# microsoft/gated-graph-neural-network-samples

Hardware: AMD Instinct MI355X
Metric: node-state updates/sec on QM9-shaped graphs, h=100, 4 edge types (higher is better)
Workload: dtype f32

## Files before the change

### gated-graph-neural-network-samples_amd/csrc/ggnn_common.h

```cpp
#pragma once
#include <hip/hip_runtime.h>
#include <atomic>
#include <cstdarg>
#include <cstdio>
#include "../../include/ggnn_hip.h"

namespace ggnn {

typedef float f32x4 __attribute__((ext_vector_type(4)));

constexpr int kNumXcd = 8;

char* error_buffer();
int fail(int code, const char* fmt, ...);

#define GGNN_CHECK_ARG(cond, ...) \
    do { if (!(cond)) return ::ggnn::fail(GGNN_E_INVALID, __VA_ARGS__); } while (0)

#define GGNN_CHECK_HIP(expr)                                                                   \
    do {                                                                                       \
        hipError_t e_ = (expr);                                                                \
        if (e_ != hipSuccess)                                                                  \
            return ::ggnn::fail(GGNN_E_HIP, "%s failed: %s", #expr, hipGetErrorString(e_));    \
    } while (0)

inline bool aligned16(const void* p) { return (reinterpret_cast<uintptr_t>(p) & 15u) == 0; }

int num_cus();

int stream_order_after(hipStream_t waiter, hipStream_t producer);

template <class Kernel>
inline hipError_t allow_dynamic_lds(Kernel* kernel, size_t bytes, std::atomic<unsigned long long>& done) {
    int dev = 0;
    if (hipError_t e = hipGetDevice(&dev); e != hipSuccess) return e;
    const unsigned long long bit = 1ULL << (dev & 63);
    if (done.load(std::memory_order_acquire) & bit) return hipSuccess;
    if (hipError_t e = hipFuncSetAttribute(reinterpret_cast<const void*>(kernel), hipFuncAttributeMaxDynamicSharedMemorySize,
                                           (int)bytes); e != hipSuccess) return e;
    done.fetch_or(bit, std::memory_order_release);
    return hipSuccess;
}

}
```

### gated-graph-neural-network-samples_amd/csrc/ggnn_gemm.hip

```cpp
#include "ggnn_gemm.hpp"

namespace ggnn {

static inline int round_up8(int x) { return (x + 7) / 8 * 8; }

constexpr int kPersistBlocksPerCU = 2;

template <int KC, int MT, int NT, int NW, class Epi>
static int launch_gemm(const GemmOperands& g, const Epi& epi, hipStream_t st) {
    using Cfg = GemmCfg<KC, MT, NT, NW>;
    const int ncg = (g.N + Cfg::BN - 1) / Cfg::BN;
    const int row_tiles = (g.M + Cfg::BM - 1) / Cfg::BM;
    if (row_tiles == 0 || ncg == 0) return GGNN_OK;
    const int nstages = g.nseg * (g.D / KC);
    int workers = round_up8(row_tiles);
    if (nstages == 1) {
        int target = num_cus() * kPersistBlocksPerCU / ncg;
        target = target / 8 * 8;
        if (target < 8) target = 8;
        if (workers > target) workers = target;
    }
    const dim3 grid((unsigned)(ncg * workers));
    hipLaunchKernelGGL((ggnn_gemm_kernel<KC, MT, NT, NW, Epi>), grid, dim3(Cfg::THREADS), Cfg::LDS_BYTES, st,
                       g, epi, ncg, row_tiles, workers);
// ... 257 lines not shown
    GGNN_CHECK_ARG(aligned16(dY) && aligned16(WT), "pointers must be 16-byte aligned");
    GemmOperands g{};
    for (int s = 0; s < nseg_y; ++s) { g.A[s] = dY + (size_t)s * D; g.lda[s] = ldy; }
    g.nseg = nseg_y; g.D = D; g.M = V;
    g.B = WT; g.ldb = K; g.b_blk_cols = K; g.b_blk_stride = 0; g.N = K;
    const int inc0 = inc ? xcols - D : xcols;
    EpiBwdDx e{dx, xcols > 0 ? xcols : 4, xcols, inc0, dinc, nin, T, use_avg, dh, D, acc_dx, acc_dh};
    return dispatch_gemm(g, e, (hipStream_t)stream);
}

extern "C" int ggnn_gru_packed_gather_f32(const float* const* x_segs, int nx, const float* h, const float* packed,
                                          const float* bg, const float* bc, float* h_out, const float* Hrows,
                                          const int32_t* row_ptr, const int32_t* gather_row, const float* nin, int T, int use_avg,
                                          int V, int D, int act, int gru_fmt, int32_t* tile_counter, ggnn_stream_t stream) {
    return ggnn_gru_packed_gather_train_f32(x_segs, nx, h, packed, bg, bc, h_out, Hrows, row_ptr, gather_row, nin, T, use_avg,
                                            nullptr, nullptr, nullptr, nullptr, V, D, act, gru_fmt, tile_counter, stream);
}

extern "C" int ggnn_gru_packed_gather_train_f32(const float* const* x_segs, int nx, const float* h, const float* packed,
                                                const float* bg, const float* bc, float* h_out, const float* Hrows,
                                                const int32_t* row_ptr, const int32_t* gather_row, const float* nin, int T,
                                                int use_avg, float* save_r, float* save_u, float* save_c, float* save_incoming,
                                                int V, int D, int act, int gru_fmt, int32_t* tile_counter, ggnn_stream_t stream) {
    if (int rc = check_common(V, D)) return rc;
    if (int rc = gru_fmt_check(gru_fmt)) return rc;
    const bool save = save_r || save_u || save_c || save_incoming;
    GGNN_CHECK_ARG(!save || (save_r && save_u && save_c && save_incoming && aligned16(save_r) && aligned16(save_u) && aligned16(save_c) &&
                             aligned16(save_incoming)), "save_r / save_u / save_c / save_incoming must be given together, 16-byte aligned");
    GGNN_CHECK_ARG(nx >= 1 && nx <= 3, "nx %d outside 1..3", nx);
    GGNN_CHECK_ARG(act == GGNN_ACT_TANH || act == GGNN_ACT_RELU, "unknown activation %d", act);
    if (!gru_fused_supported(D)) return fail(GGNN_E_UNSUPPORTED, "no fused GRU for hidden size %d", D);
    if (V == 0) return GGNN_OK;
    GGNN_CHECK_ARG(h && packed && bg && bc && h_out && h_out != h && Hrows && row_ptr && T > 0, "null pointer or h_out aliases h");
    GGNN_CHECK_ARG(!use_avg || nin, "nin is required for mean aggregation");
    GGNN_CHECK_ARG(nx == 1 || x_segs, "residual segments missing");
    GGNN_CHECK_ARG(aligned16(h) && aligned16(packed) && aligned16(bg) && aligned16(bc) && aligned16(h_out) && aligned16(Hrows),
                   "pointers must be 16-byte aligned");
    GruFusedArgs a{};
    for (int s = 0; s + 1 < nx; ++s) {
        GGNN_CHECK_ARG(x_segs[s] && aligned16(x_segs[s]) && x_segs[s] != h_out, "residual segment %d null, misaligned or aliasing h_out", s);
        a.x[s] = x_segs[s];
    }
    a.nx = nx; a.h = h; a.bg = bg; a.bc = bc; a.h_out = h_out; a.V = V; a.act = act;
    a.save_r = save_r; a.save_u = save_u; a.save_c = save_c; a.save_x = save_incoming;
    a.g_H = Hrows; a.g_row_ptr = row_ptr; a.g_idx = gather_row; a.g_nin = nin; a.g_T = T; a.g_use_avg = use_avg;
    a.tickets = tile_counter; a.fmt = gru_fmt;
    return gru_fused_dispatch(a, D, const_cast<float*>(packed), (hipStream_t)stream);
}

extern "C" int ggnn_gru_bwd_dx_cand_f32(const float* dpc, const float* WcT, const float* h, const float* r, float* dx, float* dh,
                                        float* dpg, int nx, int V, int D, ggnn_stream_t stream) {
    if (int rc = check_common(V, D)) return rc;
    GGNN_CHECK_ARG(nx >= 1 && nx <= kGemmMaxSeg - 1, "nx %d outside 1..%d", nx, kGemmMaxSeg - 1);
    if (V == 0) return GGNN_OK;
    GGNN_CHECK_ARG(dpc && WcT && h && r && dx && dh && dpg, "null pointer");
    GGNN_CHECK_ARG(aligned16(dpc) && aligned16(WcT) && aligned16(h) && aligned16(r) && aligned16(dx) && aligned16(dh) && aligned16(dpg),
                   "pointers must be 16-byte aligned");
    const int K = (nx + 1) * D;
    GemmOperands g{};
    g.A[0] = dpc; g.lda[0] = D; g.nseg = 1; g.D = D; g.M = V;
    g.B = WcT; g.ldb = K; g.b_blk_cols = K; g.b_blk_stride = 0; g.N = K;
    EpiBwdCand e{dx, nx * D, nx * D, h, r, dh, dpg, D};
    return dispatch_gemm(g, e, (hipStream_t)stream);
}

extern "C" int ggnn_gru_bwd_dx_gates_f32(const float* dpg, const float* WgT, float* dx, float* dinc, const float* nin, int T,
                                         int use_avg, float* dh, int nx, int V, int D, ggnn_stream_t stream) {
    if (int rc = check_common(V, D)) return rc;
// ... 12 lines not shown
```

### gated-graph-neural-network-samples_amd/csrc/ggnn_gemm.hpp

```cpp
#pragma once
#include "ggnn_common.h"

namespace ggnn {

constexpr int kGemmMaxSeg = 8;
constexpr int kGruFusedMaxNx = 3;

struct GemmOperands {
    const float* A[kGemmMaxSeg];
    int lda[kGemmMaxSeg];
    int nseg;
    int D;
    const float* B;
    int ldb;
    int b_blk_cols;
    long b_blk_stride;
    int M, N;
};

__device__ __forceinline__ f32x4 ld4(const float* p) { return *reinterpret_cast<const f32x4*>(p); }
__device__ __forceinline__ void st4(float* p, f32x4 v) { *reinterpret_cast<f32x4*>(p) = v; }

__device__ __forceinline__ float sigmoid_f(float x) { return __builtin_amdgcn_rcpf(1.0f + __expf(-x)); }
__device__ __forceinline__ float tanh_f(float x) { return 1.0f - 2.0f * __builtin_amdgcn_rcpf(1.0f + __expf(2.0f * x)); }
// ... 125 lines not shown
            return;
        }
        f32x4 t = v;
        if (acc_dx) t = t + ld4(dx + (size_t)row * ld_dx + col);
        if (col < inc0) { st4(dx + (size_t)row * ld_dx + col, t); return; }
        if (use_avg) {
            float deg = 0.f;
            for (int k = 0; k < T; ++k) deg += nin[(size_t)row * T + k];
            t = t / (deg + 1e-7f);
        }
        st4(dinc + (size_t)row * D + (col - inc0), t);
    }
};

struct GruFusedArgs {
    const float* x[3];
    int nx;
    const float* h;
    const float* Wg; const float* bg; const float* Wc; const float* bc;
    float* h_out; float* save_r; float* save_u; float* save_c;
    float* save_x;
    int V; int act;
    const float* g_H; const int* g_row_ptr; const int* g_idx; const float* g_nin; int g_T; int g_use_avg;
    int* tickets;
    int fmt;
    unsigned long long* tdbg;
};

int gru_fused_supported(int D);
int gru_pack_floats(int D, int nx);
int gru_fused_dispatch(const GruFusedArgs& a, int D, float* packed, hipStream_t st);

template <int KC, int MT, int NT, int NW>
struct GemmCfg {
    static constexpr int BN = NT * 16;
    static constexpr int LDB = BN + 4;
    static constexpr int BM = NW * MT * 16;
    static constexpr int NC = KC / 16;
    static constexpr int NR = (KC % 16) / 4;
    static constexpr int THREADS = NW * 64;
    static constexpr int BVEC = (KC * (BN / 4) + THREADS - 1) / THREADS;
    static constexpr size_t LDS_BYTES = (size_t)KC * LDB * sizeof(float);
};

template <int KC, int MT, int NT, int NW, class Epi>
__global__ __launch_bounds__(NW * 64) void ggnn_gemm_kernel(GemmOperands g, Epi epi, int ncg,
// ... 135 lines not shown
```

### gated-graph-neural-network-samples_amd/csrc/ggnn_gru_fused.hip

```cpp
#include "ggnn_split.hpp"
#include <type_traits>

#ifndef GGNN_COOP_DEPTH
#define GGNN_COOP_DEPTH 1
#endif
#ifndef GGNN_GRU_STAMPS
#define GGNN_GRU_STAMPS 0
#endif
#if GGNN_GRU_STAMPS
#define GGNN_TDBG(a) (a).tdbg
#else
#define GGNN_TDBG(a) ((unsigned long long*)nullptr)
#endif

#ifndef GGNN_GRU_ABLATE
#define GGNN_GRU_ABLATE 0
#endif
#if GGNN_GRU_ABLATE
#define GGNN_ABL(BIT) ((ablate & (BIT)) != 0)
#define GGNN_ABL_PARAM , int ablate
#define GGNN_ABL_ARG , gru_ablate_bits()
static int gru_ablate_bits() { static const int v = [] { const char* e = getenv("GGNN_GRU_DBG"); return e ? atoi(e) : 0; }(); return v; }
#else
#define GGNN_ABL(BIT) (false)
#define GGNN_ABL_PARAM
#define GGNN_ABL_ARG
#endif

namespace ggnn {

constexpr int kTkRuntime = -1, kTkStatic = 0, kTkCounter = 1;

int gru_panel_supported(int D);
int gru_panel_pack_floats(int D, int nx);
int gru_panel_dispatch(const GruFusedArgs& a, int D, float* packed, hipStream_t st);

int gru_split_launch(int D, int nx, bool gather, const GruFusedArgs& a, float* packed, hipStream_t st);

#ifndef GGNN_GRU_TU_SPLIT
int gru_pack_floats(int D, int nx) {
    if (gru_panel_supported(D)) return gru_panel_pack_floats(D, nx);
    const bool sp = split_matrix_path();
    static_assert(ImgCfg<100, true>::IMG >= ImgCfg<100, true, kSplitF16x2>::IMG && ImgCfg<64, true>::IMG >= ImgCfg<64, true, kSplitF16x2>::IMG &&
                  ImgCfg<32, true>::IMG >= ImgCfg<32, true, kSplitF16x2>::IMG, "bf16x3 images are the larger ones");
    switch (D) {
        case 100: return 3 * (nx + 1) * (sp ? ImgCfg<100, true>::IMG : ImgCfg<100, false>::IMG);
        case 64: return 3 * (nx + 1) * (sp ? ImgCfg<64, true>::IMG : ImgCfg<64, false>::IMG);
        case 32: return 3 * (nx + 1) * (sp ? ImgCfg<32, true>::IMG : ImgCfg<32, false>::IMG);
        default: return 0;
    }
}
#endif

template <int D, bool SPLIT, int FMT = kSplitBf16x3>
// ... 10 lines not shown
    return (pos % 3) < 2 ? 2 * (pos / 3) + (pos % 3) : 2 * (NX + 1) + pos / 3;
}

template <int FMT>
__device__ __forceinline__ f32x4 sigmoid4_acc(f32x4 z, f32x4 b_scaled) {
    constexpr float k = -kLog2e * SplitFmt<FMT>::acc_scale;
    return rcp_4(exp2_4(z * k + b_scaled) + 1.0f);
}
template <int FMT>
__device__ __forceinline__ f32x4 tanh4_acc(f32x4 z, f32x4 b_scaled) {
    constexpr float k = 2.0f * kLog2e * SplitFmt<FMT>::acc_scale;
    return 1.0f - 2.0f * rcp_4(exp2_4(z * k + b_scaled) + 1.0f);
}

template <int D>
__device__ __forceinline__ void frag_zero(Frag<D>& f) {
#pragma unroll
    for (int c = 0; c < StageCfg<D>::NC; ++c) f.v[c] = f32x4{0.f, 0.f, 0.f, 0.f};
#pragma unroll
    for (int q = 0; q < StageCfg<D>::NR; ++q) f.r[q] = 0.f;
}

template <int D>
__device__ __forceinline__ void frag_add(Frag<D>& f, const Frag<D>& t) {
#pragma unroll
    for (int c = 0; c < StageCfg<D>::NC; ++c) f.v[c] += t.v[c];
#pragma unroll
    for (int q = 0; q < StageCfg<D>::NR; ++q) f.r[q] += t.r[q];
}

template <int D, int NX, int NW, bool SAVE, bool GATHER, bool SPLIT, bool SAVEX = SAVE, int FORM = 0, int FMT = kSplitBf16x3,
          int TK = kTkRuntime, bool G4AVG = false>
__global__ __launch_bounds__(NW * 64, FORM == 1 ? 2 : 1) void ggnn_gru_fused_kernel(GruFusedArgs a, const float* __restrict__ packed GGNN_ABL_PARAM) {
    static_assert(SPLIT || FMT == kSplitBf16x3, "the f32-MFMA kernels have no operand format");
    using C = StageCfg<D>;
    using I = ImgCfg<D, SPLIT, FMT>;
    using SC = SplitCfg<D, FMT>;
    constexpr bool HALF = FORM != 0;
    constexpr bool DEEP = FORM == 2;
    constexpr int NSLOT = DEEP ? 3 : 2;
    static_assert(!HALF || SPLIT, "the half-stage forms are split-form kernels");
    static_assert(FORM != 1 || NW == 4, "form 1 is the four-wave kernel");
    static_assert(!G4AVG || GATHER, "G4AVG fixes the gather's parameters");
    auto dyn_tk = [&]() -> bool {
        if constexpr (TK == kTkRuntime) return a.tickets != nullptr;
        else return TK == kTkCounter;
    };
    constexpr int NT = C::NT, NC = C::NC, NR = C::NR;
    constexpr int NSTAGE = 3 * (NX + 1);
    constexpr int SLOT = HALF ? SC::HA : I::IMG;
    extern __shared__ __attribute__((aligned(16))) float lds_[];

    const int tid = threadIdx.x, lane = tid & 63;
    const int wave = __builtin_amdgcn_readfirstlane(tid >> 6);
    const int li = lane & 15, kq = lane >> 4;
    if (GGNN_TDBG(a) && tid == 0) {
        a.tdbg[4096 + blockIdx.x * 4 + 0] = __builtin_amdgcn_s_memtime();
        a.tdbg[4096 + blockIdx.x * 4 + 1] = __builtin_amdgcn_s_memrealtime();
    }

    const int wt_total = (a.V + 15) / 16;
    const int nb = gridDim.x;
    const int full_tk = wt_total / (NW * nb) * nb;
    const int rest = wt_total - full_tk * NW;
    const int tail_w = (rest + nb - 1) / nb;
    const int n_tk = full_tk + (tail_w ? (rest + tail_w - 1) / tail_w : 0);
    const bool coop_tail = !HALF && (tail_w == 1) && (NT <= NW);
    auto is_coop = [&](int t) -> bool { return coop_tail && t >= full_tk && t < n_tk; };
    auto tile_of = [&](int t) -> int {
        if (t < full_tk) return t * NW + wave;
        if (t >= n_tk) return -1;
        if (coop_tail) return full_tk * NW + (t - full_tk);
        const int tl = full_tk * NW + (t - full_tk) * tail_w + wave;
        return (wave < tail_w && tl < wt_total) ? tl : -1;
    };

    constexpr int BIAS_FLOATS = (4 * D + 4 + 63) / 64 * 64;
    float* bias_s = lds_;
    float* ring = lds_ + BIAS_FLOATS;
    int* tk_slot = reinterpret_cast<int*>(bias_s + 4 * D);
    constexpr int RHP = C::BN + 4;
    float* rh_x = ring + NSLOT * SLOT;
    for (int i = tid; i < 4 * D; i += NW * 64)
        bias_s[i] = i < 2 * D ? -kLog2e * a.bg[i] : (i < 3 * D ? 2.0f * kLog2e * a.bc[i - 2 * D] : a.bc[i - 3 * D]);
    const bool late = FORM == 1 || wave >= NW / 2;
    int tk = blockIdx.x, tk_next = blockIdx.x + nb;
    if (dyn_tk() && tid == 0) *tk_slot = nb + atomicAdd(a.tickets, 1);

    int cur = 0;
    auto image_src = [&](int image) -> const float* {
        const float* p = packed;
        asm volatile("" : "+s"(p));
        return p + (size_t)image * I::IMG;
    };
    auto dma = [&](const float* src, float* dst) {
        if constexpr (SPLIT) dma_image_asm<I::IMG_BYTES, NW>(src, dst, wave, lane);
        else dma_image<I::IMG_BYTES, NW>(src, dst, wave, lane);
    };
    auto publish = [&]() { if constexpr (SPLIT) dma_wait(); __syncthreads(); };
    auto dma_ha = [&](const float* src, float* dst) { dma_kib_asm<SC::HA_BYTES / 1024, NW>(src, dst, wave, lane); };
    auto dma_hb = [&](const float* src, float* dst) { dma_kib_asm<SC::HB_BYTES / 1024, NW>(src, dst, wave, lane); };
    constexpr int KA = SC::HA_BYTES / 1024, KB = SC::HB_BYTES / 1024;
    const int own_a = KA / NW + (wave < KA % NW ? 1 : 0), own_b = KB / NW + (wave < KB % NW ? 1 : 0);
    auto publish_deep = [&](int own) {
        switch (own) {
            case 0: asm volatile("s_waitcnt vmcnt(0) lgkmcnt(0)" ::: "memory"); break;
// ... 2 lines not shown
            case 3: asm volatile("s_waitcnt vmcnt(3) lgkmcnt(0)" ::: "memory"); break;
            case 4: asm volatile("s_waitcnt vmcnt(4) lgkmcnt(0)" ::: "memory"); break;
            case 5: asm volatile("s_waitcnt vmcnt(5) lgkmcnt(0)" ::: "memory"); break;
            case 6: asm volatile("s_waitcnt vmcnt(6) lgkmcnt(0)" ::: "memory"); break;
            case 7: asm volatile("s_waitcnt vmcnt(7) lgkmcnt(0)" ::: "memory"); break;
            case 8: asm volatile("s_waitcnt vmcnt(8) lgkmcnt(0)" ::: "memory"); break;
            case 9: asm volatile("s_waitcnt vmcnt(9) lgkmcnt(0)" ::: "memory"); break;
            default: asm volatile("s_waitcnt vmcnt(10) lgkmcnt(0)" ::: "memory"); break;
        }
        __builtin_amdgcn_s_barrier();
    };
    static_assert(!DEEP || (SC::HA_BYTES / 1024 + NW - 1) / NW <= 10, "publish_deep covers <= 10 pieces per wave");
    if constexpr (DEEP) {
        dma_ha(packed, ring);
        dma_hb(packed + SC::HA, ring + SLOT);
    } else if constexpr (HALF) dma_ha(packed, ring);
    else dma(packed, ring);

    constexpr int GSEG = NX - 1, GBUF = GSEG & 1;
    constexpr int KI = 4;
    constexpr int G_U = NX == 1 ? NSTAGE : 3 * (NX - 1);
    constexpr bool G_NEXT = (NX == 1);
    int g_beg = 0, g_end = 0;
    int g_i[KI] = {0, 0, 0, 0};
    f32x4 g_n = {0.f, 0.f, 0.f, 0.f};
    float g_den = 1.f, g_rcp = 1.f;
    Frag<D> gt;

    auto g_ptrs = [&](int r, bool on) {
        const int b = ldi_b(a.g_row_ptr, (unsigned)r * 4u), e = ldi_b(a.g_row_ptr, (unsigned)r * 4u + 4u);
        g_beg = on ? b : 0; g_end = on ? e : 0;
        if constexpr (G4AVG) {
            g_n = ld4_b(a.g_nin, (unsigned)r * 16u);
        } else if (a.g_use_avg) {
            if (a.g_T == 4) {
                g_n = ld4_b(a.g_nin, (unsigned)r * 16u);
            } else {
                float deg = 0.f;
                for (int t = 0; t < a.g_T; ++t) deg += a.g_nin[(size_t)r * a.g_T + t];
                g_n = f32x4{deg, 0.f, 0.f, 0.f};
            }
        }
    };
    auto touch = [](auto v) { asm volatile("" :: "v"(v)); };
    auto g_index = [&](int part) {
        if (part != 2) {
            touch(g_beg); touch(g_end);
            g_den = (((g_n.x + g_n.y) + g_n.z) + g_n.w) + 1e-7f;
            if constexpr (NX == 1) g_rcp = 1.0f / g_den;
        }
        if (part != 1) {
#pragma unroll
            for (int j = 0; j < KI; ++j) {
                g_i[j] = 0;
                if (g_beg + j < g_end) g_i[j] = ldi_b(a.g_idx, (unsigned)(g_beg + j) * 4u);
            }
        }
    };
    auto g_rows0 = [&](Frag<D>& f, int part) {
        if (part != 2) { touch(g_i[0]); touch(g_i[1]); touch(g_i[2]); touch(g_i[3]); }
        if (part != 1) {
            load_frag<D>(f, a.g_H, g_i[0], kq);
            load_frag<D>(gt, a.g_H, g_i[1], kq);
        }
    };
    auto g_rows = [&](Frag<D>& f, int k, int part) {
        if (part != 2) { if (g_beg + k - 1 < g_end) frag_add<D>(f, gt); }
        if (part != 1) load_frag<D>(gt, a.g_H, g_i[k], kq);
    };
    auto g_finish = [&](Frag<D>& f) {
        if (g_beg + KI - 1 < g_end) frag_add<D>(f, gt);
        for (int e = g_beg + KI; e < g_end; ++e) {
            load_frag<D>(gt, a.g_H, a.g_idx[e], kq);
            frag_add<D>(f, gt);
        }
        if (g_beg >= g_end) frag_zero<D>(f);
        if (G4AVG || a.g_use_avg) {
            const float den = g_den, r = g_rcp;
            auto dv = [&](float x) {
                if constexpr (NX == 1) { const float q = x * r; return fmaf(fmaf(-den, q, x), r, q); }
                else return x / den;
            };
#pragma unroll
            for (int c = 0; c < NC; ++c) f.v[c] = f32x4{dv(f.v[c].x), dv(f.v[c].y), dv(f.v[c].z), dv(f.v[c].w)};
#pragma unroll
            for (int q = 0; q < NR; ++q) f.r[q] = dv(f.r[q]);
        }
    };

    auto store_x = [&](const Frag<D>& f, int row_) {
        const unsigned ob = ((unsigned)row_ * (unsigned)D + 4u * (unsigned)kq) * 4u;
#pragma unroll
        for (int c = 0; c < NC; ++c) st4_b(a.save_x, ob + 64u * c, f.v[c]);
#pragma unroll
        for (int q = 0; q < NR; ++q) *reinterpret_cast<float*>(reinterpret_cast<char*>(a.save_x) + ob - 16u * (unsigned)kq + (16u * NC + 4u * q + (unsigned)kq) * 4u) = f.r[q];
    };
    Frag<D> hf, xf[2];
    {
        const int t0 = tile_of(tk);
        const bool on = t0 >= 0;
        const int r0 = (on ? t0 : 0) * 16 + li;
        const int r0c = r0 < a.V ? r0 : a.V - 1;
        if constexpr (GATHER) {
// ... 285 lines not shown
#pragma unroll
            for (int c = 0; c < NC; ++c) rh.v[c] = acc_r[c] * hf.v[c];
#pragma unroll
            for (int q = 0; q < NR; ++q) {
                const float t0 = __shfl(acc_r[NT - 1].x, li + 16 * q), t1 = __shfl(acc_r[NT - 1].y, li + 16 * q);
                const float t2 = __shfl(acc_r[NT - 1].z, li + 16 * q), t3 = __shfl(acc_r[NT - 1].w, li + 16 * q);
                const float rr = kq == 0 ? t0 : (kq == 1 ? t1 : (kq == 2 ? t2 : t3));
                rh.r[q] = rr * hf.r[q];
            }
        }

        if (dyn_tk() && tid == 0) tk_slot[(p + 1) & 1] = nb + tk_fetch;
        GGNN_STAGE(3 * NX + 2, acc_c, rh)
#undef GGNN_STAGE
#undef GGNN_HALF_STAGE
#undef GGNN_COOP_STAGE
        tk = tk_next;
        tk_next = dyn_tk() ? __builtin_amdgcn_readfirstlane(tk_slot[(p + 1) & 1]) : tk_next + nb;

        if constexpr (coop) {
            const int col = wave * 16 + 4 * kq;
            if (wave < NT && col < D && row < a.V && !GGNN_ABL(4)) {
                f32x4 c;
                if (a.act == GGNN_ACT_TANH) {
                    c = tanh4_acc<FMT>(acc_c[0], ld4(bias_s + 2 * D + col));
                } else {
                    c = acc_c[0] * SplitFmt<FMT>::acc_scale + ld4(bias_s + 3 * D + col);
                    c.x = fmaxf(c.x, 0.f); c.y = fmaxf(c.y, 0.f); c.z = fmaxf(c.z, 0.f); c.w = fmaxf(c.w, 0.f);
                }
                const f32x4 u = acc_u[0], hv = acc_r[0];
                st4_b(a.h_out, ((unsigned)row * D + col) * 4u, u * hv + (1.0f - u) * c);
                if constexpr (SAVE) { if (a.save_c) st4_b(a.save_c, ((unsigned)row * D + col) * 4u, c); }
            }
            return;
        }
        f32x4 hrem = {0.f, 0.f, 0.f, 0.f};
        if (active) {
            stage_tail_reduce<D>(acc_c);
            if constexpr (C::TAILPACK3) {
                constexpr int SH2 = 32 * ((D % 16) / 4);
                f32x4 ct;
                ct.x = __shfl(acc_r[NT - 1].x, lane + SH2); ct.y = __shfl(acc_r[NT - 1].y, lane + SH2);
                ct.z = __shfl(acc_r[NT - 1].z, lane + SH2); ct.w = __shfl(acc_r[NT - 1].w, lane + SH2);
                acc_c[NT - 1] = ct + acc_c[NT - 1];
            }
#pragma unroll
            for (int q = 0; q < NR; ++q) {
                const float h0 = __shfl(hf.r[q], li), h1 = __shfl(hf.r[q], li + 16);
                const float h2 = __shfl(hf.r[q], li + 32), h3 = __shfl(hf.r[q], li + 48);
                if (kq == q) hrem = f32x4{h0, h1, h2, h3};
            }
        }
        if (active && row < a.V && !GGNN_ABL(4)) {
#pragma unroll
            for (int nt = 0; nt < NT; ++nt) {
                const int col = nt * 16 + 4 * kq;
                if (col < D) {
                    f32x4 hv;
                    if (nt < NC) hv = hf.v[nt];
                    else hv = hrem;
                    f32x4 c;
                    if (a.act == GGNN_ACT_TANH) {
                        c = tanh4_acc<FMT>(acc_c[nt], ld4(bias_s + 2 * D + col));
                    } else {
                        c = acc_c[nt] * SplitFmt<FMT>::acc_scale + ld4(bias_s + 3 * D + col);
                        c.x = fmaxf(c.x, 0.f); c.y = fmaxf(c.y, 0.f); c.z = fmaxf(c.z, 0.f); c.w = fmaxf(c.w, 0.f);
                    }
                    const f32x4 u = acc_u[nt];
                    st4_b(a.h_out, ((unsigned)row * D + col) * 4u, u * hv + (1.0f - u) * c);
                    if constexpr (SAVE) { if (a.save_c) st4_b(a.save_c, ((unsigned)row * D + col) * 4u, c); }
                }
            }
        }
    };
    int p = 0;
    for (; tk < n_main; ++p) run_pass(std::false_type{}, p);
    if constexpr (!HALF) { for (; tk < n_tk; ++p) run_pass(std::true_type{}, p); }
    if (GGNN_TDBG(a) && tid == 0) {
        a.tdbg[4096 + blockIdx.x * 4 + 2] = __builtin_amdgcn_s_memtime();
        a.tdbg[4096 + blockIdx.x * 4 + 3] = __builtin_amdgcn_s_memrealtime();
    }
}

template <int D, int NX, int NW, bool SAVE, bool GATHER, bool SPLIT, bool SAVEX = SAVE, int FORM = 0, int FMT = kSplitBf16x3,
          int TK = kTkRuntime, bool G4AVG = false>
static int launch_gru_fused_m(const GruFusedArgs& a_in, float* packed, hipStream_t st) {
    using C = StageCfg<D>;
    using I = ImgCfg<D, SPLIT, FMT>;
    GruFusedArgs a = a_in;
#if GGNN_GRU_STAMPS
    { const char* e = getenv("GGNN_GRU_TPTR"); a.tdbg = e ? (unsigned long long*)strtoull(e, nullptr, 10) : nullptr; }
#endif
    if (a.Wg) {
        hipLaunchKernelGGL((gru_pack_weights_kernel<D, SPLIT, FMT>), dim3(8, 3 * (NX + 1)), dim3(256), 0, st, a.Wg, a.Wc, NX, packed);
        GGNN_CHECK_HIP(hipGetLastError());
    }
    if (a.h == nullptr) return GGNN_OK;
    if ((unsigned long long)a.V * D >= (1ULL << 30) || (a.g_H && (unsigned long long)a.V * a.g_T * D >= (1ULL << 30)))
        return fail(GGNN_E_UNSUPPORTED, "fused GRU indexes with 32-bit byte offsets: V*D (and V*T*D for the gathered rows) "
                                        "must be < 2^30 (V=%d, D=%d)", a.V, D);
    constexpr size_t bias_b = (size_t)((4 * D + 4 + 63) / 64 * 64) * sizeof(float);
    const size_t lds = FORM == 1 ? (size_t)2 * SplitCfg<D, FMT>::HA_BYTES + bias_b
                     : FORM == 2 ? (size_t)3 * SplitCfg<D, FMT>::HA_BYTES + bias_b
                                 : (size_t)2 * I::IMG_BYTES + bias_b + (size_t)16 * (C::BN + 4) * sizeof(float);
    const int wt_total = (a.V + 15) / 16;
    int nb = FORM == 1 ? 2 * num_cus() : num_cus();
    if (nb > wt_total) nb = wt_total;
    static const int coop_small = [] { const char* e = getenv("GGNN_GRU_COOP_SMALL"); return e ? atoi(e) : 1; }();
    if (FORM == 0 && coop_small && wt_total > nb && wt_total <= 2 * nb && StageCfg<D>::NT <= NW) nb = wt_total;
    static std::atomic<unsigned long long> lds_ok{0};
    if (lds > 64 * 1024) GGNN_CHECK_HIP(allow_dynamic_lds(&ggnn_gru_fused_kernel<D, NX, NW, SAVE, GATHER, SPLIT, SAVEX, FORM, FMT, TK, G4AVG>, lds, lds_ok));
    hipLaunchKernelGGL((ggnn_gru_fused_kernel<D, NX, NW, SAVE, GATHER, SPLIT, SAVEX, FORM, FMT, TK, G4AVG>), dim3(nb), dim3(NW * 64), lds, st, a, (const float*)packed GGNN_ABL_ARG);
    GGNN_CHECK_HIP(hipGetLastError());
    return GGNN_OK;
}

#ifdef GGNN_GRU_TU_SPLIT
std::atomic<int>& gru_form_override();
int gru_wide_launch(int D, int nx, int ntw_req, const GruFusedArgs& a, float* packed, hipStream_t st);
int gru_wide_supported(int D, int nx, const GruFusedArgs& a);
static int gru_form(int nx, int fmt) {
    const int v = gru_form_override().load(std::memory_order_relaxed);
    return v >= 0 ? v : ((nx >= 2 || fmt == kSplitF16x2) ? 1 : 0);
}

template <int D, int NX, int NW, int FORM, int FMT>
static int split_launch_gather(bool save, const GruFusedArgs& a, float* packed, hipStream_t st) {
    return save ? launch_gru_fused_m<D, NX, NW, true, true, true, true, FORM, FMT>(a, packed, st)
                : launch_gru_fused_m<D, NX, NW, false, true, true, false, FORM, FMT>(a, packed, st);
}
template <int D, int NX, int NW, int FORM, int FMT>
static int split_launch_hot(const GruFusedArgs& a, float* packed, hipStream_t st) {
    return a.tickets ? launch_gru_fused_m<D, NX, NW, false, true, true, false, FORM, FMT, kTkCounter, true>(a, packed, st)
                     : launch_gru_fused_m<D, NX, NW, false, true, true, false, FORM, FMT, kTkStatic, true>(a, packed, st);
}

template <int D, int FMT>
static int split_launch_d(int nx, bool save, bool gather, const GruFusedArgs& a, float* packed, hipStream_t st) {
    if constexpr (SplitCfg<D>::OK) {
        const int f = gru_form(nx, FMT);
        if (gather && (f == 6 || (f >= 60 && f < 70)) && gru_wide_supported(D, nx, a))
            return gru_wide_launch(D, nx, f >= 60 ? f - 60 : 0, a, packed, st);
        if constexpr (D == 100) {
            if (gather && !save && a.g_use_avg && a.g_T == 4) {
                if (f == 1) {
                    switch (nx) {
                        case 1: return split_launch_hot<D, 1, 4, 1, FMT>(a, packed, st);
                        case 2: return split_launch_hot<D, 2, 4, 1, FMT>(a, packed, st);
                        case 3: return split_launch_hot<D, 3, 4, 1, FMT>(a, packed, st);
                    }
                }
                if constexpr (FMT == kSplitBf16x3) { if (f == 0 && nx == 1) return split_launch_hot<D, 1, 8, 0, FMT>(a, packed, st); }
            }
        }
        if (gather && f == 2) {
            switch (nx) {
                case 1: return split_launch_gather<D, 1, 8, 2, FMT>(save, a, packed, st);
                case 2: return split_launch_gather<D, 2, 8, 2, FMT>(save, a, packed, st);
                case 3: return split_launch_gather<D, 3, 8, 2, FMT>(save, a, packed, st);
            }
        }
        if (gather && f == 1) {
            switch (nx) {
                case 1: return split_launch_gather<D, 1, 4, 1, FMT>(save, a, packed, st);
                case 2: return split_launch_gather<D, 2, 4, 1, FMT>(save, a, packed, st);
                case 3: return split_launch_gather<D, 3, 4, 1, FMT>(save, a, packed, st);
            }
// ... 18 lines not shown
    const bool save = a.save_r != nullptr;
#ifdef GGNN_PROBE_NX
#ifndef GGNN_PROBE_SAVE
#define GGNN_PROBE_SAVE true
#endif
#ifndef GGNN_PROBE_SAVEX
#define GGNN_PROBE_SAVEX GGNN_PROBE_SAVE
#endif
#ifndef GGNN_PROBE_FMT
#define GGNN_PROBE_FMT kSplitF16x2
#endif
#ifndef GGNN_PROBE_FORM
#define GGNN_PROBE_FORM 0
#endif
#ifndef GGNN_PROBE_NW
#define GGNN_PROBE_NW 8
#endif
#ifndef GGNN_PROBE_TK
#define GGNN_PROBE_TK kTkRuntime
#endif
#ifndef GGNN_PROBE_G4AVG
#define GGNN_PROBE_G4AVG false
#endif
    return launch_gru_fused_m<100, GGNN_PROBE_NX, GGNN_PROBE_NW, GGNN_PROBE_SAVE, true, true, GGNN_PROBE_SAVEX, GGNN_PROBE_FORM, GGNN_PROBE_FMT,
                              GGNN_PROBE_TK, GGNN_PROBE_G4AVG>(a, packed, st);
#else
    const bool f2 = gru_launch_fmt(a.fmt) == kSplitF16x2;
    switch (D) {
        case 100: return f2 ? split_launch_d<100, kSplitF16x2>(nx, save, gather, a, packed, st) : split_launch_d<100, kSplitBf16x3>(nx, save, gather, a, packed, st);
        case 64: return f2 ? split_launch_d<64, kSplitF16x2>(nx, save, gather, a, packed, st) : split_launch_d<64, kSplitBf16x3>(nx, save, gather, a, packed, st);
        case 32: return f2 ? split_launch_d<32, kSplitF16x2>(nx, save, gather, a, packed, st) : split_launch_d<32, kSplitBf16x3>(nx, save, gather, a, packed, st);
        default: return fail(GGNN_E_UNSUPPORTED, "no split-form fused GRU for hidden size %d", D);
    }
#endif
}
#else
template <int D, int NX, int NW, bool SAVE, bool GATHER>
static int launch_gru_fused(const GruFusedArgs& a, float* packed, hipStream_t st) {
    if (SplitCfg<D>::OK && split_matrix_path()) return gru_split_launch(D, NX, GATHER, a, packed, st);
    return launch_gru_fused_m<D, NX, NW, SAVE, GATHER, false>(a, packed, st);
}

static bool nosave_kernel() {
    static const bool v = [] { const char* e = getenv("GGNN_GRU_NOSAVE_KERNEL"); return e && atoi(e) != 0; }();
    return v;
}

template <int D>
// ... 40 lines not shown
```

### gated-graph-neural-network-samples_amd/csrc/ggnn_propagate.hip

```cpp
#include "ggnn_common.h"
#include <cstring>

static constexpr int kTileCounters = 1024;

extern "C" size_t ggnn_sparse_propagate_workspace_bytes(int V, int D, int T, int64_t compact_rows) {
    if (V < 0 || D <= 0 || T <= 0) return 0;
    const size_t vd = (size_t)V * D * sizeof(float);
    const size_t hrows = compact_rows >= 0 ? (size_t)(compact_rows > 0 ? compact_rows : 1) * D * sizeof(float)
                                           : (size_t)V * T * D * sizeof(float);
    return hrows + 3 * vd + ggnn_gru_workspace_bytes(V, D) + kTileCounters * sizeof(int32_t) + 6 * 256;
}

static inline char* bump(char*& p, size_t bytes) {
    char* r = p;
    p += (bytes + 255) / 256 * 256;
    return r;
}

extern "C" int ggnn_sparse_propagate_f32(
        const float* h0, int V, int D, int T,
        const int32_t* row_ptr, const int32_t* gather_row, const int32_t* pair_node, const int64_t* type_row_off,
        const float* nin, int use_avg,
        int num_layers, const int32_t* layer_timesteps, const int32_t* res_ptr, const int32_t* res_idx,
        const float* const* edge_w, const float* const* edge_packed, const float* const* edge_bias,
        const float* const* Wg, const float* const* bg, const float* const* Wc, const float* const* bc,
        const float* const* gru_packed, const int32_t* gru_fmt, const int32_t* edge_fmt, int act, int fuse_gather,
        float* const* layer_out, void* ws, size_t ws_bytes, ggnn_stream_t stream) {
    GGNN_CHECK_ARG(V >= 0 && D > 0 && D % 4 == 0 && T > 0, "bad sizes V=%d D=%d T=%d", V, D, T);
    GGNN_CHECK_ARG(num_layers > 0 && layer_timesteps && res_ptr && layer_out, "bad layer description");
    GGNN_CHECK_ARG(edge_w || edge_packed, "edge weights missing");
    GGNN_CHECK_ARG(bg && bc && (gru_packed || (Wg && Wc)), "GRU weights missing");
    if (V == 0) return GGNN_OK;
    GGNN_CHECK_ARG(h0 && row_ptr && ws, "null pointer");
    const bool compact = pair_node != nullptr && type_row_off != nullptr;
    const int64_t rows = compact ? type_row_off[T] : -1;
    if (ws_bytes < ggnn_sparse_propagate_workspace_bytes(V, D, T, rows))
        return ggnn::fail(GGNN_E_WORKSPACE, "propagate workspace too small: %zu < %zu", ws_bytes,
                          ggnn_sparse_propagate_workspace_bytes(V, D, T, rows));
    const size_t vd = (size_t)V * D * sizeof(float);
    char* p = reinterpret_cast<char*>((reinterpret_cast<size_t>(ws) + 255) / 256 * 256);
    float* H = reinterpret_cast<float*>(bump(p, compact ? (size_t)(rows > 0 ? rows : 1) * D * sizeof(float)
                                                       : (size_t)V * T * D * sizeof(float)));
    float* incoming = reinterpret_cast<float*>(bump(p, vd));
    float* ping[2] = {reinterpret_cast<float*>(bump(p, vd)), nullptr};
    ping[1] = reinterpret_cast<float*>(bump(p, vd));
    int32_t* counters = reinterpret_cast<int32_t*>(bump(p, kTileCounters * sizeof(int32_t)));
    void* gru_ws = p;
    const size_t gru_ws_bytes = ggnn_gru_workspace_bytes(V, D);
    int step_no = 0;
    {
        int total_steps = 0;
        for (int l = 0; l < num_layers; ++l) total_steps += layer_timesteps[l] > 0 ? layer_timesteps[l] : 0;
        if (total_steps > kTileCounters) total_steps = kTileCounters;
        if (total_steps > 0) GGNN_CHECK_HIP(hipMemsetAsync(counters, 0, (size_t)total_steps * sizeof(int32_t), (hipStream_t)stream));
    }

    const float* states[64];
    GGNN_CHECK_ARG(num_layers < 63, "too many layers");
    states[0] = h0;
    for (int l = 0; l < num_layers; ++l) {
        const int nres = res_ptr[l + 1] - res_ptr[l];
        GGNN_CHECK_ARG(nres >= 0 && nres <= 6, "layer %d has %d residual inputs (max 6)", l, nres);
        const float* xs[7];
        for (int i = 0; i < nres; ++i) {
            const int src = res_idx[res_ptr[l] + i];
            GGNN_CHECK_ARG(src >= 0 && src <= l, "layer %d: residual index %d refers to a later layer", l, src);
            xs[i] = states[src];
        }
        xs[nres] = incoming;
        const int nx = nres + 1;
        GGNN_CHECK_ARG(layer_out[l], "layer_out[%d] is null", l);
        const float* cur = states[l];
        const int steps = layer_timesteps[l];
        const float* bias_l = edge_bias ? edge_bias[l] : nullptr;
        const bool packed_gru = gru_packed && gru_packed[l] && ggnn_gru_is_fused(D) && nx <= 3;
        const int fmt_l = gru_fmt ? gru_fmt[l] : GGNN_GRU_FMT_BF16X3;
        const bool gather_in_gru = fuse_gather > 0 && nx <= fuse_gather && packed_gru && ggnn_gru_is_fused(D) == 1 && bias_l == nullptr &&
                                   (unsigned long long)V * T * D < (1ULL << 30);
        for (int s = 0; s < steps; ++s) {
            int rc;
            if (compact) {
                const bool packed = edge_packed && edge_packed[l];
                rc = ggnn_msg_transform_compact_f32(cur, packed ? nullptr : edge_w[l], pair_node, type_row_off, H,
                                                    packed ? const_cast<float*>(edge_packed[l]) : gru_ws,
                                                    packed ? ggnn_msg_transform_compact_workspace_bytes(D, T) : gru_ws_bytes,
                                                    V, D, T, (packed && edge_fmt) ? edge_fmt[l] : GGNN_GRU_FMT_BF16X3, stream);
            } else {
                GGNN_CHECK_ARG(edge_w && edge_w[l], "dense transform needs raw edge weights");
                rc = ggnn_msg_transform_f32(cur, D, edge_w[l], H, V, D, T, stream);
            }
            if (rc) return rc;
            float* out = (s + 1 == steps) ? layer_out[l] : ping[s & 1];
            static const bool dyn_tiles = [] { const char* e = getenv("GGNN_DYN_TILES"); return !e || atoi(e) != 0; }();
            int32_t* counter = (dyn_tiles && step_no < kTileCounters) ? counters + step_no : nullptr;
            ++step_no;
            if (gather_in_gru) {
                rc = ggnn_gru_packed_gather_f32(xs, nx, cur, gru_packed[l], bg[l], bc[l], out, H, row_ptr, gather_row, nin, T,
                                                use_avg, V, D, act, fmt_l, counter, stream);
            } else {
                rc = ggnn_gather_segment_sum_f32(H, row_ptr, gather_row, nin, bias_l, use_avg, incoming, V, D, T, stream);
                if (rc) return rc;
                if (packed_gru)
                    rc = ggnn_gru_packed_f32(xs, nx, cur, gru_packed[l], bg[l], bc[l], out, nullptr, nullptr, nullptr, V, D, act,
                                             fmt_l, counter, stream);
                else {
                    GGNN_CHECK_ARG(Wg && Wc && Wg[l] && Wc[l], "layer %d needs raw GRU weights (no packed images for it)", l);
                    rc = ggnn_gru_f32(xs, nx, cur, Wg[l], bg[l], Wc[l], bc[l], out, gru_ws, gru_ws_bytes, nullptr, nullptr,
                                      nullptr, V, D, act, stream);
                }
            }
            if (rc) return rc;
            cur = out;
        }
        if (steps == 0) {
            GGNN_CHECK_HIP(hipMemcpyAsync(layer_out[l], cur, vd, hipMemcpyDeviceToDevice, (hipStream_t)stream));
        }
        states[l + 1] = layer_out[l];
    }
    return GGNN_OK;
}
```

### gated-graph-neural-network-samples_amd/ops.py

```python
from __future__ import annotations

import ctypes
import os
from dataclasses import dataclass
from typing import Any, Dict, List, Optional, Sequence

import torch

from . import _lib
from ._lib import check

ACT_IDS = {"tanh": 0, "relu": 1}
GRU_FUSED_MAX_INPUTS = 3
GRU_MAX_INPUTS = 7
GRU_FMT_F16X2, GRU_FMT_EXACT = 2, 3


def kernel_width(D: int) -> int:
    D = int(D)
    if D <= 0:
        raise ValueError("hidden_size must be positive")
    if D % 32 == 0 or D % 100 == 0:
        return D
    for w in (32, 64, 100, 128, 192, 256):
# ... 999 lines not shown
    V, D = h.shape
    R = comp.num_rows
    if out is None:
        out = torch.empty((max(R, 1), D), dtype=torch.float32, device=h.device)
    off = (ctypes.c_int64 * (T + 1))(*comp.type_row_off)
    _launch("msg_transform_compact", lambda: lib.ggnn_msg_transform_compact_f32(
        _ptr(h), None, _ptr(comp.pair_node), off, _ptr(out), _ptr(packed), packed.numel() * 4, V, D, T, int(fmt), _stream()))
    return out


def _ptr_array(tensors):
    if tensors is None:
        return None
    return (ctypes.c_void_p * len(tensors))(*[None if t is None else t.data_ptr() for t in tensors])


def sparse_propagate(h0: torch.Tensor, index: MessageIndex, comp: Optional[CompactSources], nin: torch.Tensor, use_avg: bool,
                     layer_timesteps: Sequence[int], residuals: Sequence[Sequence[int]],
                     edge_w: Sequence[torch.Tensor], edge_packed: Optional[Sequence[torch.Tensor]],
                     edge_bias: Optional[Sequence[Optional[torch.Tensor]]],
                     Wg: Sequence[torch.Tensor], bg: Sequence[torch.Tensor], Wc: Sequence[torch.Tensor], bc: Sequence[torch.Tensor],
                     gru_packed: Optional[Sequence[torch.Tensor]], activation: str,
                     fuse_gather: Optional[bool] = None, gru_fmt: Optional[Sequence[int]] = None,
                     edge_fmt: Optional[Sequence[int]] = None) -> List[torch.Tensor]:
    if fuse_gather is None:
        fuse_gather = FUSE_GATHER
    lib = _lib.load()
    _req(h0, torch.float32, "h0")
    V, D = h0.shape
    T, L = index.num_edge_types, len(layer_timesteps)
    act = ACT_IDS.get(activation.lower())
    if act is None:
        raise Exception("Unknown activation function type '%s'." % activation)
    rows = comp.num_rows if comp is not None else -1
    ws_bytes = lib.ggnn_sparse_propagate_workspace_bytes(V, D, T, rows)
    ws = torch.empty(ws_bytes, dtype=torch.uint8, device=h0.device)
    outs = [torch.empty_like(h0) for _ in range(L)]
    res_ptr = [0]
    res_idx = []
    for r in residuals:
        res_idx.extend(int(i) for i in r)
        res_ptr.append(len(res_idx))
    i32 = lambda xs: (ctypes.c_int32 * max(len(xs), 1))(*xs)
    off = None if comp is None else (ctypes.c_int64 * (T + 1))(*comp.type_row_off)
    gather = index.gather_row if comp is None else comp.gather_row
    _launch("sparse_propagate", lambda: lib.ggnn_sparse_propagate_f32(
        _ptr(h0), V, D, T, _ptr(index.row_ptr), _ptr(gather), None if comp is None else _ptr(comp.pair_node), off,
        _ptr(nin), 1 if use_avg else 0, L, i32([int(x) for x in layer_timesteps]), i32(res_ptr), i32(res_idx),
        _ptr_array(edge_w), _ptr_array(edge_packed), _ptr_array(edge_bias), _ptr_array(Wg), _ptr_array(bg), _ptr_array(Wc),
        _ptr_array(bc), _ptr_array(gru_packed), None if gru_fmt is None else i32([int(f) for f in gru_fmt]),
        None if edge_fmt is None else i32([int(f) for f in edge_fmt]), act, int(fuse_gather),
        _ptr_array(outs), _ptr(ws), ws_bytes, _stream()))
    return outs


def gru_packed_gather(residual_segs: Sequence[torch.Tensor], h: torch.Tensor, packed: torch.Tensor, bg: torch.Tensor,
                      bc: torch.Tensor, H: torch.Tensor, index: MessageIndex, gather_row: Optional[torch.Tensor],
                      num_incoming_edges_per_type: Optional[torch.Tensor], activation: str = "tanh",
                      tile_counter: Optional[torch.Tensor] = None, save: Optional[dict] = None,
# ... 470 lines not shown
```

Baseline: 1.267 billion.

## Pad gather with a zero row and specialize fused GRU on tanh activation

Adds a zeroed sentinel row after the message buffer so the fused gather-GRU kernel can fill missing neighbour slots with that row's index and add unconditionally. This removes the per-edge bounds branches and the final zeroing of empty neighbourhoods, at the cost of extra loads of the zero row. The hot D=100, T=4 mean-aggregation path is now also templated on tanh activation and uses a reciprocal-based mean. The workspace layout changes to place the zero row and the tile counters together so one memset clears both. A caller can now pass a reusable workspace tensor.

```diff
diff --git a/gated-graph-neural-network-samples_amd/csrc/ggnn_common.h b/gated-graph-neural-network-samples_amd/csrc/ggnn_common.h
--- a/gated-graph-neural-network-samples_amd/csrc/ggnn_common.h
+++ b/gated-graph-neural-network-samples_amd/csrc/ggnn_common.h
@@ -42,4 +42,9 @@
     return hipSuccess;
 }
 
+int gru_packed_gather_zrow(const float* const* x_segs, int nx, const float* h, const float* packed, const float* bg, const float* bc,
+                           float* h_out, const float* Hrows, int zero_row, const int32_t* row_ptr, const int32_t* gather_row,
+                           const float* nin, int T, int use_avg, float* save_r, float* save_u, float* save_c, float* save_incoming,
+                           int V, int D, int act, int gru_fmt, int32_t* tile_counter, ggnn_stream_t stream);
+
 }
diff --git a/gated-graph-neural-network-samples_amd/csrc/ggnn_gemm.hip b/gated-graph-neural-network-samples_amd/csrc/ggnn_gemm.hip
--- a/gated-graph-neural-network-samples_amd/csrc/ggnn_gemm.hip
+++ b/gated-graph-neural-network-samples_amd/csrc/ggnn_gemm.hip
@@ -303,6 +303,14 @@
                                                 const int32_t* row_ptr, const int32_t* gather_row, const float* nin, int T,
                                                 int use_avg, float* save_r, float* save_u, float* save_c, float* save_incoming,
                                                 int V, int D, int act, int gru_fmt, int32_t* tile_counter, ggnn_stream_t stream) {
+    return ggnn::gru_packed_gather_zrow(x_segs, nx, h, packed, bg, bc, h_out, Hrows, 0, row_ptr, gather_row, nin, T, use_avg, save_r, save_u,
+                                        save_c, save_incoming, V, D, act, gru_fmt, tile_counter, stream);
+}
+
+int ggnn::gru_packed_gather_zrow(const float* const* x_segs, int nx, const float* h, const float* packed, const float* bg, const float* bc,
+                                 float* h_out, const float* Hrows, int zero_row, const int32_t* row_ptr, const int32_t* gather_row,
+                                 const float* nin, int T, int use_avg, float* save_r, float* save_u, float* save_c, float* save_incoming,
+                                 int V, int D, int act, int gru_fmt, int32_t* tile_counter, ggnn_stream_t stream) {
     if (int rc = check_common(V, D)) return rc;
     if (int rc = gru_fmt_check(gru_fmt)) return rc;
     const bool save = save_r || save_u || save_c || save_incoming;
@@ -325,6 +333,7 @@
     a.nx = nx; a.h = h; a.bg = bg; a.bc = bc; a.h_out = h_out; a.V = V; a.act = act;
     a.save_r = save_r; a.save_u = save_u; a.save_c = save_c; a.save_x = save_incoming;
     a.g_H = Hrows; a.g_row_ptr = row_ptr; a.g_idx = gather_row; a.g_nin = nin; a.g_T = T; a.g_use_avg = use_avg;
+    a.g_zrow = zero_row > 0 && (unsigned long long)(zero_row + 1) * D < (1ULL << 30) ? zero_row : 0;
     a.tickets = tile_counter; a.fmt = gru_fmt;
     return gru_fused_dispatch(a, D, const_cast<float*>(packed), (hipStream_t)stream);
 }
diff --git a/gated-graph-neural-network-samples_amd/csrc/ggnn_gemm.hpp b/gated-graph-neural-network-samples_amd/csrc/ggnn_gemm.hpp
--- a/gated-graph-neural-network-samples_amd/csrc/ggnn_gemm.hpp
+++ b/gated-graph-neural-network-samples_amd/csrc/ggnn_gemm.hpp
@@ -171,6 +171,7 @@
     float* save_x;
     int V; int act;
     const float* g_H; const int* g_row_ptr; const int* g_idx; const float* g_nin; int g_T; int g_use_avg;
+    int g_zrow;
     int* tickets;
     int fmt;
     unsigned long long* tdbg;
diff --git a/gated-graph-neural-network-samples_amd/csrc/ggnn_gru_fused.hip b/gated-graph-neural-network-samples_amd/csrc/ggnn_gru_fused.hip
--- a/gated-graph-neural-network-samples_amd/csrc/ggnn_gru_fused.hip
+++ b/gated-graph-neural-network-samples_amd/csrc/ggnn_gru_fused.hip
@@ -30,6 +30,7 @@
 namespace ggnn {
 
 constexpr int kTkRuntime = -1, kTkStatic = 0, kTkCounter = 1;
+constexpr int kActRuntime = -1;
 
 int gru_panel_supported(int D);
 int gru_panel_pack_floats(int D, int nx);
@@ -86,6 +87,14 @@
 }
 
 template <int D>
+__device__ __forceinline__ void frag_pin(Frag<D>& f) {
+#pragma unroll
+    for (int c = 0; c < StageCfg<D>::NC; ++c) { asm volatile("" : "+v"(f.v[c].x), "+v"(f.v[c].y), "+v"(f.v[c].z), "+v"(f.v[c].w)); }
+#pragma unroll
+    for (int q = 0; q < StageCfg<D>::NR; ++q) asm volatile("" : "+v"(f.r[q]));
+}
+
+template <int D>
 __device__ __forceinline__ void frag_add(Frag<D>& f, const Frag<D>& t) {
 #pragma unroll
     for (int c = 0; c < StageCfg<D>::NC; ++c) f.v[c] += t.v[c];
@@ -94,7 +103,7 @@
 }
 
 template <int D, int NX, int NW, bool SAVE, bool GATHER, bool SPLIT, bool SAVEX = SAVE, int FORM = 0, int FMT = kSplitBf16x3,
-          int TK = kTkRuntime, bool G4AVG = false>
+          int TK = kTkRuntime, bool G4AVG = false, bool ZROW = false, int ACT = kActRuntime>
 __global__ __launch_bounds__(NW * 64, FORM == 1 ? 2 : 1) void ggnn_gru_fused_kernel(GruFusedArgs a, const float* __restrict__ packed GGNN_ABL_PARAM) {
     static_assert(SPLIT || FMT == kSplitBf16x3, "the f32-MFMA kernels have no operand format");
     using C = StageCfg<D>;
@@ -106,6 +115,13 @@
     static_assert(!HALF || SPLIT, "the half-stage forms are split-form kernels");
     static_assert(FORM != 1 || NW == 4, "form 1 is the four-wave kernel");
     static_assert(!G4AVG || GATHER, "G4AVG fixes the gather's parameters");
+    static_assert(!ZROW || (GATHER && !SAVEX), "ZROW is a property of the gather-fused inference launches");
+    static_assert(ACT == kActRuntime || ACT == GGNN_ACT_TANH, "only tanh is fixed at compile time");
+    auto act_tanh = [&]() -> bool {
+        if constexpr (ACT == kActRuntime) return a.act == GGNN_ACT_TANH;
+        else return true;
+    };
+    constexpr bool RCP_MEAN = NX == 1 || G4AVG;
     auto dyn_tk = [&]() -> bool {
         if constexpr (TK == kTkRuntime) return a.tickets != nullptr;
         else return TK == kTkCounter;
@@ -145,7 +161,7 @@
     int* tk_slot = reinterpret_cast<int*>(bias_s + 4 * D);
     constexpr int RHP = C::BN + 4;
     float* rh_x = ring + NSLOT * SLOT;
-    for (int i = tid; i < 4 * D; i += NW * 64)
+    for (int i = tid; i < (ACT == GGNN_ACT_TANH ? 3 : 4) * D; i += NW * 64)
         bias_s[i] = i < 2 * D ? -kLog2e * a.bg[i] : (i < 3 * D ? 2.0f * kLog2e * a.bc[i - 2 * D] : a.bc[i - 3 * D]);
     const bool late = FORM == 1 || wave >= NW / 2;
     int tk = blockIdx.x, tk_next = blockIdx.x + nb;
@@ -194,7 +210,8 @@
     constexpr int G_U = NX == 1 ? NSTAGE : 3 * (NX - 1);
     constexpr bool G_NEXT = (NX == 1);
     int g_beg = 0, g_end = 0;
-    int g_i[KI] = {0, 0, 0, 0};
+    const int g_miss = ZROW ? a.g_zrow : 0;
+    int g_i[KI] = {g_miss, g_miss, g_miss, g_miss};
     f32x4 g_n = {0.f, 0.f, 0.f, 0.f};
     float g_den = 1.f, g_rcp = 1.f;
     Frag<D> gt;
@@ -219,12 +236,12 @@
         if (part != 2) {
             touch(g_beg); touch(g_end);
             g_den = (((g_n.x + g_n.y) + g_n.z) + g_n.w) + 1e-7f;
-            if constexpr (NX == 1) g_rcp = 1.0f / g_den;
+            if constexpr (RCP_MEAN) g_rcp = 1.0f / g_den;
         }
         if (part != 1) {
 #pragma unroll
             for (int j = 0; j < KI; ++j) {
-                g_i[j] = 0;
+                g_i[j] = g_miss;
                 if (g_beg + j < g_end) g_i[j] = ldi_b(a.g_idx, (unsigned)(g_beg + j) * 4u);
             }
         }
@@ -237,20 +254,23 @@
         }
     };
     auto g_rows = [&](Frag<D>& f, int k, int part) {
-        if (part != 2) { if (g_beg + k - 1 < g_end) frag_add<D>(f, gt); }
+        if (part != 2) {
+            if (ZROW || g_beg + k - 1 < g_end) frag_add<D>(f, gt);
+            if constexpr (ZROW) frag_pin<D>(f);
+        }
         if (part != 1) load_frag<D>(gt, a.g_H, g_i[k], kq);
     };
     auto g_finish = [&](Frag<D>& f) {
-        if (g_beg + KI - 1 < g_end) frag_add<D>(f, gt);
+        if (ZROW || g_beg + KI - 1 < g_end) frag_add<D>(f, gt);
         for (int e = g_beg + KI; e < g_end; ++e) {
             load_frag<D>(gt, a.g_H, a.g_idx[e], kq);
             frag_add<D>(f, gt);
         }
-        if (g_beg >= g_end) frag_zero<D>(f);
+        if constexpr (!ZROW) { if (g_beg >= g_end) frag_zero<D>(f); }
         if (G4AVG || a.g_use_avg) {
             const float den = g_den, r = g_rcp;
             auto dv = [&](float x) {
-                if constexpr (NX == 1) { const float q = x * r; return fmaf(fmaf(-den, q, x), r, q); }
+                if constexpr (RCP_MEAN) { const float q = x * r; return fmaf(fmaf(-den, q, x), r, q); }
                 else return x / den;
             };
 #pragma unroll
@@ -582,7 +602,7 @@
             const int col = wave * 16 + 4 * kq;
             if (wave < NT && col < D && row < a.V && !GGNN_ABL(4)) {
                 f32x4 c;
-                if (a.act == GGNN_ACT_TANH) {
+                if (act_tanh()) {
                     c = tanh4_acc<FMT>(acc_c[0], ld4(bias_s + 2 * D + col));
                 } else {
                     c = acc_c[0] * SplitFmt<FMT>::acc_scale + ld4(bias_s + 3 * D + col);
@@ -620,7 +640,7 @@
                     if (nt < NC) hv = hf.v[nt];
                     else hv = hrem;
                     f32x4 c;
-                    if (a.act == GGNN_ACT_TANH) {
+                    if (act_tanh()) {
                         c = tanh4_acc<FMT>(acc_c[nt], ld4(bias_s + 2 * D + col));
                     } else {
                         c = acc_c[nt] * SplitFmt<FMT>::acc_scale + ld4(bias_s + 3 * D + col);
@@ -643,7 +663,7 @@
 }
 
 template <int D, int NX, int NW, bool SAVE, bool GATHER, bool SPLIT, bool SAVEX = SAVE, int FORM = 0, int FMT = kSplitBf16x3,
-          int TK = kTkRuntime, bool G4AVG = false>
+          int TK = kTkRuntime, bool G4AVG = false, bool ZROW = false, int ACT = kActRuntime>
 static int launch_gru_fused_m(const GruFusedArgs& a_in, float* packed, hipStream_t st) {
     using C = StageCfg<D>;
     using I = ImgCfg<D, SPLIT, FMT>;
@@ -669,8 +689,8 @@
     static const int coop_small = [] { const char* e = getenv("GGNN_GRU_COOP_SMALL"); return e ? atoi(e) : 1; }();
     if (FORM == 0 && coop_small && wt_total > nb && wt_total <= 2 * nb && StageCfg<D>::NT <= NW) nb = wt_total;
     static std::atomic<unsigned long long> lds_ok{0};
-    if (lds > 64 * 1024) GGNN_CHECK_HIP(allow_dynamic_lds(&ggnn_gru_fused_kernel<D, NX, NW, SAVE, GATHER, SPLIT, SAVEX, FORM, FMT, TK, G4AVG>, lds, lds_ok));
-    hipLaunchKernelGGL((ggnn_gru_fused_kernel<D, NX, NW, SAVE, GATHER, SPLIT, SAVEX, FORM, FMT, TK, G4AVG>), dim3(nb), dim3(NW * 64), lds, st, a, (const float*)packed GGNN_ABL_ARG);
+    if (lds > 64 * 1024) GGNN_CHECK_HIP(allow_dynamic_lds(&ggnn_gru_fused_kernel<D, NX, NW, SAVE, GATHER, SPLIT, SAVEX, FORM, FMT, TK, G4AVG, ZROW, ACT>, lds, lds_ok));
+    hipLaunchKernelGGL((ggnn_gru_fused_kernel<D, NX, NW, SAVE, GATHER, SPLIT, SAVEX, FORM, FMT, TK, G4AVG, ZROW, ACT>), dim3(nb), dim3(NW * 64), lds, st, a, (const float*)packed GGNN_ABL_ARG);
     GGNN_CHECK_HIP(hipGetLastError());
     return GGNN_OK;
 }
@@ -691,8 +711,9 @@
 }
 template <int D, int NX, int NW, int FORM, int FMT>
 static int split_launch_hot(const GruFusedArgs& a, float* packed, hipStream_t st) {
-    return a.tickets ? launch_gru_fused_m<D, NX, NW, false, true, true, false, FORM, FMT, kTkCounter, true>(a, packed, st)
-                     : launch_gru_fused_m<D, NX, NW, false, true, true, false, FORM, FMT, kTkStatic, true>(a, packed, st);
+    if (a.tickets && a.g_zrow > 0) return launch_gru_fused_m<D, NX, NW, false, true, true, false, FORM, FMT, kTkCounter, true, true, GGNN_ACT_TANH>(a, packed, st);
+    return a.tickets ? launch_gru_fused_m<D, NX, NW, false, true, true, false, FORM, FMT, kTkCounter, true, false, GGNN_ACT_TANH>(a, packed, st)
+                     : launch_gru_fused_m<D, NX, NW, false, true, true, false, FORM, FMT, kTkStatic, true, false, GGNN_ACT_TANH>(a, packed, st);
 }
 
 template <int D, int FMT>
@@ -702,7 +723,7 @@
         if (gather && (f == 6 || (f >= 60 && f < 70)) && gru_wide_supported(D, nx, a))
             return gru_wide_launch(D, nx, f >= 60 ? f - 60 : 0, a, packed, st);
         if constexpr (D == 100) {
-            if (gather && !save && a.g_use_avg && a.g_T == 4) {
+            if (gather && !save && a.g_use_avg && a.g_T == 4 && a.act == GGNN_ACT_TANH) {
                 if (f == 1) {
                     switch (nx) {
                         case 1: return split_launch_hot<D, 1, 4, 1, FMT>(a, packed, st);
@@ -767,8 +788,14 @@
 #ifndef GGNN_PROBE_G4AVG
 #define GGNN_PROBE_G4AVG false
 #endif
+#ifndef GGNN_PROBE_ZROW
+#define GGNN_PROBE_ZROW false
+#endif
+#ifndef GGNN_PROBE_ACT
+#define GGNN_PROBE_ACT kActRuntime
+#endif
     return launch_gru_fused_m<100, GGNN_PROBE_NX, GGNN_PROBE_NW, GGNN_PROBE_SAVE, true, true, GGNN_PROBE_SAVEX, GGNN_PROBE_FORM, GGNN_PROBE_FMT,
-                              GGNN_PROBE_TK, GGNN_PROBE_G4AVG>(a, packed, st);
+                              GGNN_PROBE_TK, GGNN_PROBE_G4AVG, GGNN_PROBE_ZROW, GGNN_PROBE_ACT>(a, packed, st);
 #else
     const bool f2 = gru_launch_fmt(a.fmt) == kSplitF16x2;
     switch (D) {
diff --git a/gated-graph-neural-network-samples_amd/csrc/ggnn_propagate.hip b/gated-graph-neural-network-samples_amd/csrc/ggnn_propagate.hip
--- a/gated-graph-neural-network-samples_amd/csrc/ggnn_propagate.hip
+++ b/gated-graph-neural-network-samples_amd/csrc/ggnn_propagate.hip
@@ -8,7 +8,7 @@
     const size_t vd = (size_t)V * D * sizeof(float);
     const size_t hrows = compact_rows >= 0 ? (size_t)(compact_rows > 0 ? compact_rows : 1) * D * sizeof(float)
                                            : (size_t)V * T * D * sizeof(float);
-    return hrows + 3 * vd + ggnn_gru_workspace_bytes(V, D) + kTileCounters * sizeof(int32_t) + 6 * 256;
+    return hrows + (size_t)17 * D * sizeof(float) + 256 + 3 * vd + ggnn_gru_workspace_bytes(V, D) + kTileCounters * sizeof(int32_t) + 6 * 256;
 }
 
 static inline char* bump(char*& p, size_t bytes) {
@@ -39,12 +39,17 @@
                           ggnn_sparse_propagate_workspace_bytes(V, D, T, rows));
     const size_t vd = (size_t)V * D * sizeof(float);
     char* p = reinterpret_cast<char*>((reinterpret_cast<size_t>(ws) + 255) / 256 * 256);
-    float* H = reinterpret_cast<float*>(bump(p, compact ? (size_t)(rows > 0 ? rows : 1) * D * sizeof(float)
-                                                       : (size_t)V * T * D * sizeof(float)));
+    const size_t h_rows = compact ? (size_t)(rows > 0 ? rows : 1) : (size_t)V * T;
+    const size_t row_bytes = (size_t)D * sizeof(float);
+    const size_t z_index = (h_rows + 15) / 16 * 16;
+    const size_t zrow_span = (row_bytes + 255) / 256 * 256;
+    float* H = reinterpret_cast<float*>(bump(p, z_index * row_bytes + zrow_span + kTileCounters * sizeof(int32_t)));
+    float* zrow = H + z_index * D;
+    int32_t* counters = reinterpret_cast<int32_t*>(reinterpret_cast<char*>(zrow) + zrow_span);
+    const int zero_row = z_index < (size_t)0x7fffffff ? (int)z_index : 0;
     float* incoming = reinterpret_cast<float*>(bump(p, vd));
     float* ping[2] = {reinterpret_cast<float*>(bump(p, vd)), nullptr};
     ping[1] = reinterpret_cast<float*>(bump(p, vd));
-    int32_t* counters = reinterpret_cast<int32_t*>(bump(p, kTileCounters * sizeof(int32_t)));
     void* gru_ws = p;
     const size_t gru_ws_bytes = ggnn_gru_workspace_bytes(V, D);
     int step_no = 0;
@@ -52,7 +57,7 @@
         int total_steps = 0;
         for (int l = 0; l < num_layers; ++l) total_steps += layer_timesteps[l] > 0 ? layer_timesteps[l] : 0;
         if (total_steps > kTileCounters) total_steps = kTileCounters;
-        if (total_steps > 0) GGNN_CHECK_HIP(hipMemsetAsync(counters, 0, (size_t)total_steps * sizeof(int32_t), (hipStream_t)stream));
+        GGNN_CHECK_HIP(hipMemsetAsync(zrow, 0, zrow_span + (size_t)total_steps * sizeof(int32_t), (hipStream_t)stream));
     }
 
     const float* states[64];
@@ -95,8 +100,8 @@
             int32_t* counter = (dyn_tiles && step_no < kTileCounters) ? counters + step_no : nullptr;
             ++step_no;
             if (gather_in_gru) {
-                rc = ggnn_gru_packed_gather_f32(xs, nx, cur, gru_packed[l], bg[l], bc[l], out, H, row_ptr, gather_row, nin, T,
-                                                use_avg, V, D, act, fmt_l, counter, stream);
+                rc = ggnn::gru_packed_gather_zrow(xs, nx, cur, gru_packed[l], bg[l], bc[l], out, H, zero_row, row_ptr, gather_row, nin, T,
+                                                  use_avg, nullptr, nullptr, nullptr, nullptr, V, D, act, fmt_l, counter, stream);
             } else {
                 rc = ggnn_gather_segment_sum_f32(H, row_ptr, gather_row, nin, bias_l, use_avg, incoming, V, D, T, stream);
                 if (rc) return rc;
diff --git a/gated-graph-neural-network-samples_amd/ops.py b/gated-graph-neural-network-samples_amd/ops.py
--- a/gated-graph-neural-network-samples_amd/ops.py
+++ b/gated-graph-neural-network-samples_amd/ops.py
@@ -1045,7 +1045,7 @@
                      Wg: Sequence[torch.Tensor], bg: Sequence[torch.Tensor], Wc: Sequence[torch.Tensor], bc: Sequence[torch.Tensor],
                      gru_packed: Optional[Sequence[torch.Tensor]], activation: str,
                      fuse_gather: Optional[bool] = None, gru_fmt: Optional[Sequence[int]] = None,
-                     edge_fmt: Optional[Sequence[int]] = None) -> List[torch.Tensor]:
+                     edge_fmt: Optional[Sequence[int]] = None, ws: Optional[torch.Tensor] = None) -> List[torch.Tensor]:
     if fuse_gather is None:
         fuse_gather = FUSE_GATHER
     lib = _lib.load()
@@ -1057,7 +1057,11 @@
         raise Exception("Unknown activation function type '%s'." % activation)
     rows = comp.num_rows if comp is not None else -1
     ws_bytes = lib.ggnn_sparse_propagate_workspace_bytes(V, D, T, rows)
-    ws = torch.empty(ws_bytes, dtype=torch.uint8, device=h0.device)
+    if ws is None:
+        ws = torch.empty(ws_bytes, dtype=torch.uint8, device=h0.device)
+    else:
+        _req(ws, torch.uint8, "ws")
+        ws_bytes = ws.numel()
     outs = [torch.empty_like(h0) for _ in range(L)]
     res_ptr = [0]
     res_idx = []
```

Measured after the change: 1.278 billion, median of 6. About the same (+0.8%).
